# pakozm/lua-mapreduce

Hardware: AMD Instinct MI355X
Metric: words/sec (higher is better)
Workload: dtype u8-text/i64-counts; 1 GPU; model=europarl-wordcount, global_batch=49158635, seq_len=49158635, parallelism=dp1, splits_per_gpu=197, partitions=1, partitioner=hash-mulhi, ingestion=resident-hbm

## Files before the change

### mapreduce_amd/ops/hip/ops_ext.hip

```cpp

#include <ATen/hip/HIPContext.h>
#include <torch/extension.h>

#include <limits>
#include <map>
#include <mutex>
#include <utility>

#include "extract_sorted.hip"
#include "gradsum.hip"
#include "group.hip"
#include "join.hip"
#include "lex_order.hip"
#include "mr_kernels.hip"
#include "postings_phrase.hip"
#include "postings_query.hip"
#include "radix_sort.hip"
#include "seg_scan.hip"
#include "token_ordinals.hip"

namespace {

constexpr int kBlock = 256;
constexpr long kMaxBlocks = 2048;

long grid_for(long n, long per_thread = 1) {
  long want = (n + (long)kBlock * per_thread - 1) / ((long)kBlock * per_thread);
  if (want < 1) want = 1;
  return want < kMaxBlocks ? want : kMaxBlocks;
}

hipStream_t cur_stream() { return at::hip::getCurrentHIPStream(); }

constexpr int kTokWavesPerCu = 16;

struct TokOccupancy {
  int blocks_per_cu = 0;
  int cus = 0;
};

TokOccupancy tok_occupancy(const void* kfn, int blockn) {
  static std::mutex mu;
  static std::map<std::pair<const void*, int>, TokOccupancy> cache;
  int dev = 0;
  C10_HIP_CHECK(hipGetDevice(&dev));
  std::lock_guard<std::mutex> lock(mu);
  auto it = cache.find({kfn, dev});
  if (it != cache.end()) return it->second;
  TokOccupancy o;
  C10_HIP_CHECK(hipOccupancyMaxActiveBlocksPerMultiprocessor(
      &o.blocks_per_cu, kfn, blockn, 0));
  C10_HIP_CHECK(hipDeviceGetAttribute(
      &o.cus, hipDeviceAttributeMultiprocessorCount, dev));
  TORCH_CHECK(o.blocks_per_cu > 0 && o.cus > 0,
              "tokenizer occupancy query returned ", o.blocks_per_cu,
              " blocks/CU on ", o.cus, " CUs");
  cache[{kfn, dev}] = o;
  return o;
}

template <typename K>
long tok_grid(K kfn, int blockn, long n, long tile_bytes) {
  long tiles = (n + tile_bytes - 1) / tile_bytes;
  if (tiles < 1) tiles = 1;
  TokOccupancy o = tok_occupancy(reinterpret_cast<const void*>(kfn), blockn);
  int per_cu = kTokWavesPerCu / (blockn / WAVE);
  if (per_cu > o.blocks_per_cu) per_cu = o.blocks_per_cu;
  long resident = (long)per_cu * o.cus;
  long blocks = tiles < resident ? tiles : resident;
  return blocks < kMaxBlocks ? blocks : kMaxBlocks;
}

int rs_items() {
  static int v = -1;
  if (v < 0) {
    const char* e = getenv("MR_RS_ITEMS");
    const char* v1 = getenv("MR_RADIX_V1");
    v = (e && atoi(e) == 4 && !(v1 && v1[0] == '1')) ? 4 : 8;
  }
  return v;
}

long rs_tile() { return (long)RS_BLOCK * rs_items(); }

bool radix_v1_forced() {
  const char* v = getenv("MR_RADIX_V1");
  return v && v[0] == '1';
}

void launch_radix_hist(const u64* kin, long n, int shift, long ntiles,
                       i64* hist) {
  auto kfn = rs_items() == 4 ? radix_hist_kernel<4> : radix_hist_kernel<8>;
  hipLaunchKernelGGL(kfn, dim3(ntiles), dim3(RS_BLOCK), 0, cur_stream(),
                     kin, n, shift, ntiles, hist);
}

void launch_radix_scatter(const u64* kin, const u64* vin, long n, int shift,
                          long ntiles, const i64* base, u64* kout,
                          u64* vout) {
  static int use_v1 = -1;
  if (use_v1 < 0) use_v1 = radix_v1_forced() ? 1 : 0;
  if (use_v1)
    hipLaunchKernelGGL(radix_scatter_kernel, dim3(ntiles), dim3(RS_BLOCK), 0,
                       cur_stream(), kin, vin, n, shift, ntiles, base, kout,
                       vout);
  else {
    auto kfn = rs_items() == 4 ? radix_scatter_v2_kernel<4>
                               : radix_scatter_v2_kernel<8>;
    hipLaunchKernelGGL(kfn, dim3(ntiles), dim3(RS_BLOCK),
                       0, cur_stream(), kin, vin, n, shift, ntiles, base,
                       kout, vout);
  }
}

void launch_radix_scatter32(const u64* kin, const u32* vin, long n,
                            int shift, long ntiles, const i64* base,
                            u64* kout, u32* vout) {
  auto kfn = rs_items() == 4 ? radix_scatter_v2_kernel<4, u32>
                             : radix_scatter_v2_kernel<8, u32>;
  hipLaunchKernelGGL(kfn, dim3(ntiles), dim3(RS_BLOCK), 0, cur_stream(),
                     kin, vin, n, shift, ntiles, base, kout, vout);
}

template <bool SKIP>
void launch_bucketize_hist(const u64* kin, long n, int shift, long ntiles,
                           u32* hist) {
  auto kfn = rs_items() == 4 ? radix_hist_kernel<4, SKIP, u32>
                             : radix_hist_kernel<8, SKIP, u32>;
  hipLaunchKernelGGL(kfn, dim3(ntiles), dim3(RS_BLOCK), 0, cur_stream(),
                     kin, n, shift, ntiles, hist);
}

template <typename VT, bool SKIP>
void launch_bucketize_scatter(const u64* kin, const VT* vin, long n,
                              int shift, long ntiles, const u32* base,
                              u64* kout, VT* vout) {
  auto kfn = rs_items() == 4 ? radix_scatter_v2_kernel<4, VT, SKIP, u32>
                             : radix_scatter_v2_kernel<8, VT, SKIP, u32>;
  hipLaunchKernelGGL(kfn, dim3(ntiles), dim3(RS_BLOCK), 0, cur_stream(),
                     kin, vin, n, shift, ntiles, base, kout, vout);
}

u64* u64p(torch::Tensor& t) { return reinterpret_cast<u64*>(t.data_ptr<i64>()); }
const u64* u64cp(const torch::Tensor& t) {
  return reinterpret_cast<const u64*>(t.data_ptr<i64>());
}

void check_dev_i64(const torch::Tensor& t, const char* name) {
  TORCH_CHECK(t.is_cuda(), name, " must be on GPU");
  TORCH_CHECK(t.scalar_type() == torch::kInt64, name, " must be int64");
  TORCH_CHECK(t.is_contiguous(), name, " must be contiguous");
}

}

std::vector<torch::Tensor> tokenize(torch::Tensor text, long cap) {
  TORCH_CHECK(text.is_cuda() && text.scalar_type() == torch::kUInt8 &&
              text.is_contiguous(), "text must be contiguous u8 on GPU");
  long n = text.numel();
  auto opts = torch::TensorOptions().device(text.device()).dtype(torch::kInt64);
  auto out_hash = torch::empty({cap}, opts);
  auto out_pos = torch::empty({cap}, opts);
  auto counter = torch::zeros({1}, opts);
  long blocks = grid_for(n, TOK_BYTES);
  hipLaunchKernelGGL(tokenize_kernel, dim3(blocks), dim3(kBlock), 0,
                     cur_stream(), text.data_ptr<u8>(), n, u64p(out_hash),
                     u64p(out_pos),
                     reinterpret_cast<unsigned long long*>(counter.data_ptr<i64>()),
                     cap);
  return {out_hash, out_pos, counter};
}

void tokenize_count(torch::Tensor text, long pos_base, torch::Tensor tkeys,
                    torch::Tensor tvals, torch::Tensor texm,
                    torch::Tensor nwords) {
  TORCH_CHECK(text.is_cuda() && text.scalar_type() == torch::kUInt8 &&
              text.is_contiguous(), "text must be contiguous u8 on GPU");
  long n = text.numel();
  long cap = tkeys.numel();
  TORCH_CHECK((cap & (cap - 1)) == 0, "table capacity must be a power of 2");
  if (!n) return;
  hipLaunchKernelGGL(tokenize_count_kernel, dim3(grid_for(n, TOK_BYTES)),
                     dim3(kBlock), 0, cur_stream(), text.data_ptr<u8>(), n,
                     (u64)pos_base, u64p(tkeys), tvals.data_ptr<i64>(),
                     texm.numel() ? u64p(texm) : nullptr, (u64)(cap - 1),
                     reinterpret_cast<unsigned long long*>(nwords.data_ptr<i64>()));
}

std::vector<torch::Tensor> tokenize_spill_v2(torch::Tensor text,
                                             long pos_base, long cap) {
  TORCH_CHECK(text.is_cuda() && text.scalar_type() == torch::kUInt8 &&
              text.is_contiguous(), "text must be contiguous u8 on GPU");
  long n = text.numel();
  auto opts = torch::TensorOptions().device(text.device()).dtype(torch::kInt64);
  auto out_hash = torch::empty({cap}, opts);
  auto out_pos = torch::empty({cap}, opts);
  auto counter = torch::zeros({1}, opts);
  auto nwords = torch::zeros({1}, opts);
  if (n) {
    auto dummy = torch::empty({16}, opts);
    hipLaunchKernelGGL((tokenize_v6_kernel<16, false, 4096, 0, true>),
                       dim3(grid_for(n, TOK_BYTES)), dim3(kBlock), 0,
                       cur_stream(), text.data_ptr<u8>(), n, (u64)pos_base,
                       u64p(dummy), dummy.data_ptr<i64>(), nullptr,
                       (u64)15, u64p(out_hash), u64p(out_pos),
                       reinterpret_cast<unsigned long long*>(counter.data_ptr<i64>()),
                       cap,
                       reinterpret_cast<unsigned long long*>(nwords.data_ptr<i64>()),
                       nullptr, (const i64*)nullptr, 0, 0L);
  }
  return {out_hash, out_pos, counter, nwords};
}

std::vector<torch::Tensor> tokenize_spill_composite(
    torch::Tensor text, long pos_base, long cap, torch::Tensor split_off,
    long doc_base) {
  TORCH_CHECK(text.is_cuda() && text.scalar_type() == torch::kUInt8 &&
              text.is_contiguous(), "text must be contiguous u8 on GPU");
  check_dev_i64(split_off, "split_off");
  long n = text.numel();
  auto opts = torch::TensorOptions().device(text.device()).dtype(torch::kInt64);
  auto out_hash = torch::empty({cap}, opts);
  auto out_pos = torch::empty({cap}, opts);
  auto counter = torch::zeros({1}, opts);
  auto nwords = torch::zeros({1}, opts);
  if (n) {
    auto dummy = torch::empty({16}, opts);
    hipLaunchKernelGGL((tokenize_v6_kernel<16, false, 4096, 0, true, true>),
                       dim3(grid_for(n, TOK_BYTES)), dim3(kBlock), 0,
                       cur_stream(), text.data_ptr<u8>(), n, (u64)pos_base,
                       u64p(dummy), dummy.data_ptr<i64>(), nullptr,
                       (u64)15, u64p(out_hash), u64p(out_pos),
                       reinterpret_cast<unsigned long long*>(counter.data_ptr<i64>()),
                       cap,
                       reinterpret_cast<unsigned long long*>(nwords.data_ptr<i64>()),
                       nullptr, split_off.data_ptr<i64>(),
                       (int)split_off.numel(), doc_base);
  }
  return {out_hash, out_pos, counter, nwords};
}

void tokenize_cache_spill_composite(
    torch::Tensor text, long pos_base, torch::Tensor tkeys,
    torch::Tensor tvals, torch::Tensor texm, long spill_cap,
    torch::Tensor nwords, torch::Tensor out_hash, torch::Tensor out_pos,
    torch::Tensor counter, torch::Tensor split_off, long doc_base) {
  TORCH_CHECK(text.is_cuda() && text.scalar_type() == torch::kUInt8 &&
              text.is_contiguous(), "text must be contiguous u8 on GPU");
  check_dev_i64(split_off, "split_off");
  long n = text.numel();
  long cap = tkeys.numel();
  TORCH_CHECK((cap & (cap - 1)) == 0, "table capacity must be a power of 2");
  TORCH_CHECK(out_hash.numel() >= spill_cap && out_pos.numel() >= spill_cap,
              "spill arrays too small");
  if (!n) return;
  auto kfn =
      tokenize_v6_kernel<2048, true, 4096, 0, false, true, 2048, 0, 256>;
  long blocks = tok_grid(kfn, kBlock, n, 4096);
  static torch::Tensor cpos_gc;
  long need = blocks * 2048;
  if (!cpos_gc.defined() || cpos_gc.numel() < need ||
      cpos_gc.device() != text.device())
    cpos_gc = torch::empty({need}, torch::TensorOptions()
                                        .device(text.device())
                                        .dtype(torch::kInt64));
  hipLaunchKernelGGL(
      kfn, dim3(blocks), dim3(kBlock), 0, cur_stream(), text.data_ptr<u8>(), n,
      (u64)pos_base, u64p(tkeys), tvals.data_ptr<i64>(),
      texm.numel() ? u64p(texm) : nullptr, (u64)(cap - 1), u64p(out_hash),
      u64p(out_pos),
      reinterpret_cast<unsigned long long*>(counter.data_ptr<i64>()),
      spill_cap,
      reinterpret_cast<unsigned long long*>(nwords.data_ptr<i64>()),
      u64p(cpos_gc), split_off.data_ptr<i64>(), (int)split_off.numel(),
      doc_base);
}

std::vector<torch::Tensor> tokenize_spill(torch::Tensor text, long pos_base,
                                          long cap) {
  TORCH_CHECK(text.is_cuda() && text.scalar_type() == torch::kUInt8 &&
              text.is_contiguous(), "text must be contiguous u8 on GPU");
  long n = text.numel();
  auto opts = torch::TensorOptions().device(text.device()).dtype(torch::kInt64);
  auto out_hash = torch::empty({cap}, opts);
  auto out_pos = torch::empty({cap}, opts);
  auto counter = torch::zeros({1}, opts);
  if (n)
    hipLaunchKernelGGL(tokenize_spill_kernel, dim3(grid_for(n, TOK_BYTES)),
                       dim3(kBlock), 0, cur_stream(), text.data_ptr<u8>(), n,
                       (u64)pos_base, u64p(out_hash), u64p(out_pos),
                       reinterpret_cast<unsigned long long*>(counter.data_ptr<i64>()),
                       cap);
  return {out_hash, out_pos, counter};
}

void tokenize_cache_spill(
    torch::Tensor text, long pos_base, torch::Tensor tkeys,
    torch::Tensor tvals, torch::Tensor texm, long spill_cap,
    torch::Tensor nwords, torch::Tensor out_hash, torch::Tensor out_pos,
    torch::Tensor counter) {
  TORCH_CHECK(text.is_cuda() && text.scalar_type() == torch::kUInt8 &&
              text.is_contiguous(), "text must be contiguous u8 on GPU");
  long n = text.numel();
  long cap = tkeys.numel();
  TORCH_CHECK((cap & (cap - 1)) == 0, "table capacity must be a power of 2");
  TORCH_CHECK(out_hash.numel() >= spill_cap && out_pos.numel() >= spill_cap,
              "spill arrays too small");
  if (n) {
    const char* v = getenv("MR_TOKENIZE_V5");
    const char* v4 = getenv("MR_TOKENIZE_V4");
    if (!(v && v[0] == '1') && !(v4 && v4[0] == '1')) {
      const char* cs = getenv("MR_TOK_CACHE");
      int cache = cs ? atoi(cs) : 2048;
      const char* gp = getenv("MR_TOK_GPOS");
      bool gpos = !(gp && gp[0] == '0');
      const char* ts = getenv("MR_TOK_TILE");
      int tsz = ts ? atoi(ts) : 4096;
      const char* sc = getenv("MR_SPILL_CHUNK");
      int schunk = sc ? atoi(sc) : 2048;
      const char* tb = getenv("MR_TOK_BLOCK");
      int blockn = (tb && atoi(tb) == 512) ? 512 : 256;
      if (blockn == 512) tsz = 8192;
      auto kfn = tokenize_v6_kernel<2048, false, 4096>;
      if (gpos && blockn == 512)
        kfn = tokenize_v6_kernel<2048, true, 8192, 0, false, false, 2048,
                                 0, 512>;
      else if (gpos && tsz == 8192) kfn = tokenize_v6_kernel<2048, true, 8192>;
      else if (gpos && cache == 4096) kfn = tokenize_v6_kernel<4096, true, 4096>;
      else if (gpos && cache == 1024) kfn = tokenize_v6_kernel<1024, true, 4096>;
      else if (gpos && schunk == 128)
        kfn = tokenize_v6_kernel<2048, true, 4096, 0, false, false, 128>;
      else if (gpos && schunk == 1024)
        kfn = tokenize_v6_kernel<2048, true, 4096, 0, false, false, 1024>;
      else if (gpos && schunk == 2048)
        kfn = tokenize_v6_kernel<2048, true, 4096, 0, false, false, 2048>;
      else if (gpos && schunk == 4096)
        kfn = tokenize_v6_kernel<2048, true, 4096, 0, false, false, 4096>;
      else if (gpos) kfn = tokenize_v6_kernel<2048, true, 4096>;
      else if (cache == 512) kfn = tokenize_v6_kernel<512, false, 4096>;
      else if (cache == 1024) kfn = tokenize_v6_kernel<1024, false, 4096>;
      else if (schunk == 128)
        kfn = tokenize_v6_kernel<2048, false, 4096, 0, false, false, 128>;
      long blocks = tok_grid(kfn, blockn, n, tsz);
      static torch::Tensor cpos_g;
      u64* cpg = nullptr;
      if (gpos) {
        long need = blocks * (cache > 2048 ? cache : 2048);
        if (!cpos_g.defined() || cpos_g.numel() < need ||
            cpos_g.device() != text.device())
          cpos_g = torch::empty({need},
                                torch::TensorOptions().device(text.device())
                                    .dtype(torch::kInt64));
        cpg = u64p(cpos_g);
      }
      hipLaunchKernelGGL(kfn,
                         dim3(blocks), dim3(blockn), 0,
                         cur_stream(), text.data_ptr<u8>(), n, (u64)pos_base,
                         u64p(tkeys), tvals.data_ptr<i64>(),
                         texm.numel() ? u64p(texm) : nullptr, (u64)(cap - 1),
                         u64p(out_hash), u64p(out_pos),
                         reinterpret_cast<unsigned long long*>(counter.data_ptr<i64>()),
                         spill_cap,
                         reinterpret_cast<unsigned long long*>(nwords.data_ptr<i64>()),
                         cpg, (const i64*)nullptr, 0, 0L);
    } else if (!(v && v[0] == '1'))
      hipLaunchKernelGGL(tokenize_cache_spill_kernel,
                         dim3(grid_for(n, TOK_BYTES)), dim3(kBlock), 0,
                         cur_stream(), text.data_ptr<u8>(), n, (u64)pos_base,
                         u64p(tkeys), tvals.data_ptr<i64>(),
                         texm.numel() ? u64p(texm) : nullptr, (u64)(cap - 1),
                         u64p(out_hash), u64p(out_pos),
                         reinterpret_cast<unsigned long long*>(counter.data_ptr<i64>()),
                         spill_cap,
                         reinterpret_cast<unsigned long long*>(nwords.data_ptr<i64>()));
    else
      hipLaunchKernelGGL(tokenize_v5_kernel,
                         dim3(grid_for(n, TOK_BYTES)), dim3(kBlock), 0,
                         cur_stream(), text.data_ptr<u8>(), n, (u64)pos_base,
                         u64p(tkeys), tvals.data_ptr<i64>(),
                         texm.numel() ? u64p(texm) : nullptr, (u64)(cap - 1),
                         u64p(out_hash), u64p(out_pos),
                         reinterpret_cast<unsigned long long*>(counter.data_ptr<i64>()),
                         spill_cap,
                         reinterpret_cast<unsigned long long*>(nwords.data_ptr<i64>()));
  }
}

void tokenize_cache_spill_bucketed(
    torch::Tensor text, long pos_base, torch::Tensor tkeys,
    torch::Tensor tvals, torch::Tensor texm, long spill_bcap,
    torch::Tensor nwords, torch::Tensor out_hash, torch::Tensor out_pos,
    torch::Tensor counters) {
  TORCH_CHECK(text.is_cuda() && text.scalar_type() == torch::kUInt8 &&
              text.is_contiguous(), "text must be contiguous u8 on GPU");
  long n = text.numel();
  long cap = tkeys.numel();
  TORCH_CHECK((cap & (cap - 1)) == 0, "table capacity must be a power of 2");
  TORCH_CHECK(counters.numel() >= 256, "counters must hold 256 buckets");
  TORCH_CHECK(out_hash.numel() >= 256 * spill_bcap &&
              out_pos.numel() >= 256 * spill_bcap, "spill arrays too small");
  if (!n) return;
  const char* gp = getenv("MR_TOK_GPOS");
  bool gpos = !(gp && gp[0] == '0');
  auto kfn = tokenize_v6_kernel<2048, false, 4096, 0, false, false, 512, 256>;
  if (gpos)
    kfn = tokenize_v6_kernel<2048, true, 4096, 0, false, false, 512, 256>;
  long blocks = tok_grid(kfn, kBlock, n, 4096);
  static torch::Tensor cpos_gb;
  u64* cpg = nullptr;
  if (gpos) {
    long need = blocks * 2048;
    if (!cpos_gb.defined() || cpos_gb.numel() < need ||
        cpos_gb.device() != text.device())
      cpos_gb = torch::empty({need},
                             torch::TensorOptions().device(text.device())
                                 .dtype(torch::kInt64));
    cpg = u64p(cpos_gb);
  }
  hipLaunchKernelGGL(kfn, dim3(blocks), dim3(kBlock), 0, cur_stream(),
                     text.data_ptr<u8>(), n, (u64)pos_base, u64p(tkeys),
                     tvals.data_ptr<i64>(),
                     texm.numel() ? u64p(texm) : nullptr, (u64)(cap - 1),
                     u64p(out_hash), u64p(out_pos),
                     reinterpret_cast<unsigned long long*>(counters.data_ptr<i64>()),
                     spill_bcap,
                     reinterpret_cast<unsigned long long*>(nwords.data_ptr<i64>()),
                     cpg, (const i64*)nullptr, 0, 0L);
}

double tok6_ablate(torch::Tensor text, long mode, long iters) {
  long n = text.numel();
  auto opts = torch::TensorOptions().device(text.device()).dtype(torch::kInt64);
  long tcap = 1 << 19;
  auto tkeys = torch::full({tcap}, -1, opts);
  auto tvals = torch::zeros({tcap}, opts);
  auto texm = torch::zeros({tcap}, opts);
  long cap = n / 2 + 16;
  auto oh = torch::empty({cap}, opts);
  auto op = torch::empty({cap}, opts);
  auto ctr = torch::zeros({1}, opts);
  auto nw = torch::zeros({1}, opts);
// ... 1203 lines not shown
```

### mapreduce_amd/ops/hip/radix_sort.hip

```cpp

#include "common.h"

#define RS_BLOCK 256
#define RS_WAVES (RS_BLOCK / WAVE)
#define RS_ITEMS 8
#define RS_TILE (RS_BLOCK * RS_ITEMS)
#define RS_BINS 256

template <bool SKIP>
DEV bool rs_live(u64 k) { return !SKIP || k != HT_EMPTY; }

template <int ITEMS, bool SKIP = false, typename HT = i64>
__global__ __launch_bounds__(RS_BLOCK) void radix_hist_kernel(
    const u64* __restrict__ keys, long n, int shift, long ntiles,
    HT* __restrict__ hist) {
  __shared__ u32 lh[RS_BINS];
  for (int b = threadIdx.x; b < RS_BINS; b += blockDim.x) lh[b] = 0;
  __syncthreads();
  long tile = blockIdx.x;
  long base = tile * (RS_BLOCK * ITEMS);
  for (int r = 0; r < ITEMS; ++r) {
    long i = base + r * RS_BLOCK + threadIdx.x;
    if (i < n) {
      u64 k = keys[i];
      if (rs_live<SKIP>(k)) atomicAdd(&lh[(u32)((k >> shift) & 0xFF)], 1u);
    }
  }
  __syncthreads();
  for (int b = threadIdx.x; b < RS_BINS; b += blockDim.x)
    hist[(long)b * ntiles + tile] = (HT)lh[b];
}

template <int ITEMS, typename VT = u64, bool SKIP = false, typename BT = i64>
__global__ __launch_bounds__(RS_BLOCK) void radix_scatter_v2_kernel(
    const u64* __restrict__ keys, const VT* __restrict__ vals, long n,
    int shift, long ntiles, const BT* __restrict__ base_dx,
    u64* __restrict__ okeys, VT* __restrict__ ovals) {
  __shared__ u32 wavecnt[RS_WAVES][RS_BINS];
  __shared__ u32 cnt_base[RS_BINS];
  __shared__ u32 digit_start[RS_BINS + 1];
  __shared__ u64 stage_k[(RS_BLOCK * ITEMS)];
  __shared__ VT stage_v[(RS_BLOCK * ITEMS)];
  for (int b = threadIdx.x; b < RS_BINS; b += blockDim.x) cnt_base[b] = 0;
  long tile = blockIdx.x;
  long tbase = tile * (RS_BLOCK * ITEMS);
  long tile_n = n - tbase < (RS_BLOCK * ITEMS) ? n - tbase : (RS_BLOCK * ITEMS);
  int wave = threadIdx.x / WAVE;
  int lane = threadIdx.x % WAVE;
  u64 lt_mask = ((u64)1 << lane) - 1;
  bool has_vals = ovals != nullptr;

  __syncthreads();
  for (int r = 0; r < ITEMS; ++r) {
    long i = tbase + (long)r * RS_BLOCK + threadIdx.x;
    if (i < n) {
      u64 k = keys[i];
      if (rs_live<SKIP>(k))
        atomicAdd(&cnt_base[(u32)((k >> shift) & 0xFF)], 1u);
    }
  }
  __syncthreads();
  if (threadIdx.x == 0) {
    u32 run = 0;
    for (int d = 0; d < RS_BINS; ++d) {
      digit_start[d] = run;
      run += cnt_base[d];
    }
    digit_start[RS_BINS] = run;
  }
  __syncthreads();
  for (int b = threadIdx.x; b < RS_BINS; b += blockDim.x) cnt_base[b] = 0;
  __syncthreads();

  for (int r = 0; r < ITEMS; ++r) {
    for (int b = threadIdx.x; b < RS_BINS; b += blockDim.x)
      for (int w = 0; w < RS_WAVES; ++w) wavecnt[w][b] = 0;
    __syncthreads();
    long i = tbase + (long)r * RS_BLOCK + threadIdx.x;
    bool valid = i < n;
    u64 k = valid ? keys[i] : 0;
    valid = valid && rs_live<SKIP>(k);
    u32 d = valid ? (u32)((k >> shift) & 0xFF) : 0;
    u64 m = __ballot(valid);
    #pragma unroll
    for (int b = 0; b < 8; ++b) {
      u64 bb = __ballot(valid && ((d >> b) & 1));
      m &= ((d >> b) & 1) ? bb : ~bb;
    }
    u32 lane_rank = 0;
    if (valid) {
      lane_rank = (u32)__popcll(m & lt_mask);
      int leader = __ffsll((unsigned long long)m) - 1;
      if (lane == leader) wavecnt[wave][d] = (u32)__popcll(m);
    }
    __syncthreads();
    if (threadIdx.x < RS_BINS) {
      u32 run = cnt_base[threadIdx.x];
      #pragma unroll
      for (int w = 0; w < RS_WAVES; ++w) {
        u32 c = wavecnt[w][threadIdx.x];
        wavecnt[w][threadIdx.x] = run;
        run += c;
      }
      cnt_base[threadIdx.x] = run;
    }
    __syncthreads();
    if (valid) {
      u32 s = digit_start[d] + wavecnt[wave][d] + lane_rank;
      stage_k[s] = k;
      if (has_vals) stage_v[s] = vals[i];
    }
    __syncthreads();
  }

  long nstage = SKIP ? (long)digit_start[RS_BINS] : tile_n;
  for (long s = threadIdx.x; s < nstage; s += blockDim.x) {
    u64 k = stage_k[s];
    u32 d = (u32)((k >> shift) & 0xFF);
    u32 local = (u32)s - digit_start[d];
    long pos = (long)base_dx[(long)d * ntiles + tile] + local;
    okeys[pos] = k;
    if (has_vals) ovals[pos] = stage_v[s];
  }
}

__global__ __launch_bounds__(RS_BLOCK) void radix_scatter_kernel(
    const u64* __restrict__ keys, const u64* __restrict__ vals, long n,
    int shift, long ntiles, const i64* __restrict__ base_dx,
    u64* __restrict__ okeys, u64* __restrict__ ovals) {
  __shared__ u32 wavecnt[RS_WAVES][RS_BINS];
  __shared__ u32 cnt_base[RS_BINS];
  for (int b = threadIdx.x; b < RS_BINS; b += blockDim.x) cnt_base[b] = 0;
  long tile = blockIdx.x;
  long tbase = tile * RS_TILE;
  int wave = threadIdx.x / WAVE;
  int lane = threadIdx.x % WAVE;
  u64 lt_mask = ((u64)1 << lane) - 1;

  for (int r = 0; r < RS_ITEMS; ++r) {
    for (int b = threadIdx.x; b < RS_BINS; b += blockDim.x)
      for (int w = 0; w < RS_WAVES; ++w) wavecnt[w][b] = 0;
    __syncthreads();

    long i = tbase + (long)r * RS_BLOCK + threadIdx.x;
    bool valid = i < n;
    u64 k = valid ? keys[i] : 0;
    u32 d = valid ? (u32)((k >> shift) & 0xFF) : 0;

    u64 m = __ballot(valid);
    #pragma unroll
    for (int b = 0; b < 8; ++b) {
      u64 bb = __ballot(valid && ((d >> b) & 1));
      m &= ((d >> b) & 1) ? bb : ~bb;
    }
    u32 lane_rank = 0;
    if (valid) {
      lane_rank = (u32)__popcll(m & lt_mask);
      int leader = __ffsll((unsigned long long)m) - 1;
      if (lane == leader) wavecnt[wave][d] = (u32)__popcll(m);
    }
    __syncthreads();

    if (threadIdx.x < RS_BINS) {
      u32 run = cnt_base[threadIdx.x];
      #pragma unroll
      for (int w = 0; w < RS_WAVES; ++w) {
        u32 c = wavecnt[w][threadIdx.x];
        wavecnt[w][threadIdx.x] = run;
        run += c;
      }
      cnt_base[threadIdx.x] = run;
    }
    __syncthreads();

    if (valid) {
      u32 tile_rank = wavecnt[wave][d] + lane_rank;
      long pos = base_dx[(long)d * ntiles + tile] + tile_rank;
      okeys[pos] = k;
      if (ovals) ovals[pos] = vals[i];
    }
    __syncthreads();
  }
}

#define RS_SCAN_UNROLL 4

DEV u32 wave_incl_scan_u32(u32 v, int lane) {
  #pragma unroll
  for (int off = 1; off < WAVE; off <<= 1) {
    u32 o = __shfl_up(v, off, WAVE);
    if (lane >= off) v += o;
  }
  return v;
}

__global__ __launch_bounds__(RS_BLOCK) void rs_row_totals_kernel(
    const u32* __restrict__ hist, long ntiles, i64* __restrict__ totals) {
  __shared__ i64 wsum[RS_WAVES];
  const u32* row = hist + (long)blockIdx.x * ntiles;
  i64 acc = 0;
  for (long t0 = threadIdx.x; t0 < ntiles; t0 += RS_SCAN_UNROLL * RS_BLOCK) {
    u32 v[RS_SCAN_UNROLL];
    #pragma unroll
    for (int j = 0; j < RS_SCAN_UNROLL; ++j) {
      long t = t0 + (long)j * RS_BLOCK;
      v[j] = t < ntiles ? row[t] : 0;
    }
    #pragma unroll
    for (int j = 0; j < RS_SCAN_UNROLL; ++j) acc += v[j];
  }
  acc = wave_sum_i64(acc);
  if (threadIdx.x % WAVE == 0) wsum[threadIdx.x / WAVE] = acc;
  __syncthreads();
  if (threadIdx.x == 0) {
    i64 s = 0;
    for (int w = 0; w < RS_WAVES; ++w) s += wsum[w];
    totals[blockIdx.x] = s;
  }
}

__global__ __launch_bounds__(RS_BLOCK) void rs_row_scan_kernel(
    u32* __restrict__ hist, long ntiles, const i64* __restrict__ totals,
    i64* __restrict__ bucket_off) {
  __shared__ i64 wsum[RS_WAVES];
  __shared__ u32 wpre[RS_SCAN_UNROLL * RS_WAVES];
  __shared__ i64 row_base;
  int d = blockIdx.x;
  int wave = threadIdx.x / WAVE;
  int lane = threadIdx.x % WAVE;
  i64 tv = totals[threadIdx.x];
  i64 part = wave_sum_i64(threadIdx.x < d ? tv : 0);
  if (lane == 0) wsum[wave] = part;
  __syncthreads();
  if (threadIdx.x == 0) {
    i64 s = 0;
    for (int w = 0; w < RS_WAVES; ++w) s += wsum[w];
    row_base = s;
    bucket_off[d] = s;
    if (d == RS_BINS - 1) bucket_off[RS_BINS] = s + totals[d];
  }
  __syncthreads();
  u32 carry = (u32)row_base;
  u32* row = hist + (long)d * ntiles;
  for (long t0 = 0; t0 < ntiles; t0 += RS_SCAN_UNROLL * RS_BLOCK) {
    u32 v[RS_SCAN_UNROLL], inc[RS_SCAN_UNROLL];
    #pragma unroll
    for (int j = 0; j < RS_SCAN_UNROLL; ++j) {
      long t = t0 + (long)j * RS_BLOCK + threadIdx.x;
      v[j] = t < ntiles ? row[t] : 0;
    }
    #pragma unroll
    for (int j = 0; j < RS_SCAN_UNROLL; ++j) {
      inc[j] = wave_incl_scan_u32(v[j], lane);
      if (lane == WAVE - 1) wpre[j * RS_WAVES + wave] = inc[j];
    }
    __syncthreads();
    u32 run = carry;
    #pragma unroll
    for (int j = 0; j < RS_SCAN_UNROLL; ++j) {
      #pragma unroll
      for (int w = 0; w < RS_WAVES; ++w) {
        if (w == wave) {
          long t = t0 + (long)j * RS_BLOCK + threadIdx.x;
          if (t < ntiles) row[t] = run + inc[j] - v[j];
        }
        run += wpre[j * RS_WAVES + w];
      }
    }
    carry = run;
    __syncthreads();
  }
}

__global__ __launch_bounds__(256) void gather_i64_u32_kernel(
    const i64* __restrict__ vals, const u32* __restrict__ idx, long n,
    i64* __restrict__ out) {
  long i = (long)blockIdx.x * blockDim.x + threadIdx.x;
  long stride = (long)gridDim.x * blockDim.x;
  for (; i < n; i += stride) out[i] = vals[idx[i]];
}
```

Measured before the change: 42.60 billion words/s.

## Add single-pass register-resident radix scatter kernel and vectorized histogram loads

Adds a v3 radix scatter kernel that loads all tile keys into registers once and ranks them per wave with ballot-based match masks. Each thread owns one digit for the block-wide scan, and the kernel stages the keys in shared memory sorted by digit so the global writes land contiguously. This replaces the v2 kernel's repeated per-round block barriers and its second read of the keys. The bucketize histogram also gains a 16-byte vector load path for full, aligned tiles. The old behaviour stays available through MR_RADIX_V2=1. The cost is higher register and LDS pressure, which could lower occupancy.

Result: faster. 49.33 billion words/s (median of 6 runs) (+15.8%).

```diff
diff --git a/mapreduce_amd/ops/hip/ops_ext.hip b/mapreduce_amd/ops/hip/ops_ext.hip
--- a/mapreduce_amd/ops/hip/ops_ext.hip
+++ b/mapreduce_amd/ops/hip/ops_ext.hip
@@ -88,6 +88,22 @@
   return v && v[0] == '1';
 }
 
+bool radix_v2_forced() {
+  static int f = -1;
+  if (f < 0) {
+    const char* v = getenv("MR_RADIX_V2");
+    f = (v && v[0] == '1') ? 1 : 0;
+  }
+  return f == 1;
+}
+
+#define RS_STAGED_SCATTER(VT, SKIP, BT, LATE)                              \
+  (radix_v2_forced()                                                       \
+       ? (rs_items() == 4 ? radix_scatter_v2_kernel<4, VT, SKIP, BT>       \
+                          : radix_scatter_v2_kernel<8, VT, SKIP, BT>)      \
+       : (rs_items() == 4 ? radix_scatter_v3_kernel<4, VT, SKIP, BT, LATE> \
+                          : radix_scatter_v3_kernel<8, VT, SKIP, BT, LATE>))
+
 void launch_radix_hist(const u64* kin, long n, int shift, long ntiles,
                        i64* hist) {
   auto kfn = rs_items() == 4 ? radix_hist_kernel<4> : radix_hist_kernel<8>;
@@ -105,8 +121,7 @@
                        cur_stream(), kin, vin, n, shift, ntiles, base, kout,
                        vout);
   else {
-    auto kfn = rs_items() == 4 ? radix_scatter_v2_kernel<4>
-                               : radix_scatter_v2_kernel<8>;
+    auto kfn = RS_STAGED_SCATTER(u64, false, i64, true);
     hipLaunchKernelGGL(kfn, dim3(ntiles), dim3(RS_BLOCK),
                        0, cur_stream(), kin, vin, n, shift, ntiles, base,
                        kout, vout);
@@ -116,8 +131,7 @@
 void launch_radix_scatter32(const u64* kin, const u32* vin, long n,
                             int shift, long ntiles, const i64* base,
                             u64* kout, u32* vout) {
-  auto kfn = rs_items() == 4 ? radix_scatter_v2_kernel<4, u32>
-                             : radix_scatter_v2_kernel<8, u32>;
+  auto kfn = RS_STAGED_SCATTER(u32, false, i64, true);
   hipLaunchKernelGGL(kfn, dim3(ntiles), dim3(RS_BLOCK), 0, cur_stream(),
                      kin, vin, n, shift, ntiles, base, kout, vout);
 }
@@ -125,8 +139,11 @@
 template <bool SKIP>
 void launch_bucketize_hist(const u64* kin, long n, int shift, long ntiles,
                            u32* hist) {
-  auto kfn = rs_items() == 4 ? radix_hist_kernel<4, SKIP, u32>
-                             : radix_hist_kernel<8, SKIP, u32>;
+  auto kfn = rs_items() == 4 ? radix_hist_kernel<4, SKIP, u32, true>
+                             : radix_hist_kernel<8, SKIP, u32, true>;
+  if (radix_v2_forced())
+    kfn = rs_items() == 4 ? radix_hist_kernel<4, SKIP, u32>
+                          : radix_hist_kernel<8, SKIP, u32>;
   hipLaunchKernelGGL(kfn, dim3(ntiles), dim3(RS_BLOCK), 0, cur_stream(),
                      kin, n, shift, ntiles, hist);
 }
@@ -135,8 +152,7 @@
 void launch_bucketize_scatter(const u64* kin, const VT* vin, long n,
                               int shift, long ntiles, const u32* base,
                               u64* kout, VT* vout) {
-  auto kfn = rs_items() == 4 ? radix_scatter_v2_kernel<4, VT, SKIP, u32>
-                             : radix_scatter_v2_kernel<8, VT, SKIP, u32>;
+  auto kfn = RS_STAGED_SCATTER(VT, SKIP, u32, false);
   hipLaunchKernelGGL(kfn, dim3(ntiles), dim3(RS_BLOCK), 0, cur_stream(),
                      kin, vin, n, shift, ntiles, base, kout, vout);
 }
diff --git a/mapreduce_amd/ops/hip/radix_sort.hip b/mapreduce_amd/ops/hip/radix_sort.hip
--- a/mapreduce_amd/ops/hip/radix_sort.hip
+++ b/mapreduce_amd/ops/hip/radix_sort.hip
@@ -10,7 +10,7 @@
 template <bool SKIP>
 DEV bool rs_live(u64 k) { return !SKIP || k != HT_EMPTY; }
 
-template <int ITEMS, bool SKIP = false, typename HT = i64>
+template <int ITEMS, bool SKIP = false, typename HT = i64, bool WIDE = false>
 __global__ __launch_bounds__(RS_BLOCK) void radix_hist_kernel(
     const u64* __restrict__ keys, long n, int shift, long ntiles,
     HT* __restrict__ hist) {
@@ -19,11 +19,26 @@
   __syncthreads();
   long tile = blockIdx.x;
   long base = tile * (RS_BLOCK * ITEMS);
-  for (int r = 0; r < ITEMS; ++r) {
-    long i = base + r * RS_BLOCK + threadIdx.x;
-    if (i < n) {
-      u64 k = keys[i];
-      if (rs_live<SKIP>(k)) atomicAdd(&lh[(u32)((k >> shift) & 0xFF)], 1u);
+  if (WIDE && base + RS_BLOCK * ITEMS <= n &&
+      ((unsigned long long)keys & 15) == 0) {
+    const ulonglong2* p = reinterpret_cast<const ulonglong2*>(keys + base);
+    ulonglong2 q[ITEMS / 2];
+    #pragma unroll
+    for (int j = 0; j < ITEMS / 2; ++j) q[j] = p[j * RS_BLOCK + threadIdx.x];
+    #pragma unroll
+    for (int j = 0; j < ITEMS / 2; ++j) {
+      if (rs_live<SKIP>(q[j].x))
+        atomicAdd(&lh[(u32)((q[j].x >> shift) & 0xFF)], 1u);
+      if (rs_live<SKIP>(q[j].y))
+        atomicAdd(&lh[(u32)((q[j].y >> shift) & 0xFF)], 1u);
+    }
+  } else {
+    for (int r = 0; r < ITEMS; ++r) {
+      long i = base + r * RS_BLOCK + threadIdx.x;
+      if (i < n) {
+        u64 k = keys[i];
+        if (rs_live<SKIP>(k)) atomicAdd(&lh[(u32)((k >> shift) & 0xFF)], 1u);
+      }
     }
   }
   __syncthreads();
@@ -124,6 +139,145 @@
   }
 }
 
+DEV u32 wave_incl_scan_u32(u32 v, int lane) {
+  #pragma unroll
+  for (int off = 1; off < WAVE; off <<= 1) {
+    u32 o = __shfl_up(v, off, WAVE);
+    if (lane >= off) v += o;
+  }
+  return v;
+}
+
+template <int ITEMS, typename VT = u64, bool SKIP = false, typename BT = i64,
+          bool LATE = false>
+__global__ __launch_bounds__(RS_BLOCK) void radix_scatter_v3_kernel(
+    const u64* __restrict__ keys, const VT* __restrict__ vals, long n,
+    int shift, long ntiles, const BT* __restrict__ base_dx,
+    u64* __restrict__ okeys, VT* __restrict__ ovals) {
+  static_assert(RS_BLOCK == RS_BINS, "thread b owns digit b");
+  __shared__ u32 wcnt[RS_WAVES][RS_BINS];
+  __shared__ BT gbase[RS_BINS];
+  __shared__ u64 stage_k[(RS_BLOCK * ITEMS)];
+  __shared__ VT stage_v[(RS_BLOCK * ITEMS)];
+  long tile = blockIdx.x;
+  long tbase = tile * (RS_BLOCK * ITEMS);
+  long tile_n = n - tbase < (RS_BLOCK * ITEMS) ? n - tbase : (RS_BLOCK * ITEMS);
+  int wave = threadIdx.x / WAVE;
+  int lane = threadIdx.x % WAVE;
+  u64 lt_mask = ((u64)1 << lane) - 1;
+  bool has_vals = ovals != nullptr;
+
+  BT my_base = base_dx[(long)threadIdx.x * ntiles + tile];
+  long i0 = tbase + (long)(wave * ITEMS) * WAVE + lane;
+  u64 k[ITEMS];
+  VT v[ITEMS];
+  bool valid[ITEMS];
+  #pragma unroll
+  for (int r = 0; r < ITEMS; ++r) {
+    long i = i0 + (long)r * WAVE;
+    k[r] = keys[i < n ? i : n - 1];
+  }
+  if (has_vals && !LATE) {
+    #pragma unroll
+    for (int r = 0; r < ITEMS; ++r) {
+      long i = i0 + (long)r * WAVE;
+      v[r] = vals[i < n ? i : n - 1];
+    }
+  } else {
+    #pragma unroll
+    for (int r = 0; r < ITEMS; ++r) v[r] = 0;
+  }
+  #pragma unroll
+  for (int r = 0; r < ITEMS; ++r)
+    valid[r] = i0 + (long)r * WAVE < n && rs_live<SKIP>(k[r]);
+
+  #pragma unroll
+  for (int b = lane; b < RS_BINS; b += WAVE) wcnt[wave][b] = 0;
+  __builtin_amdgcn_fence(__ATOMIC_ACQ_REL, "wavefront");
+  __builtin_amdgcn_wave_barrier();
+  u32 rank[ITEMS];
+  #pragma unroll
+  for (int r = 0; r < ITEMS; ++r) {
+    u32 d = valid[r] ? (u32)((k[r] >> shift) & 0xFF) : 0;
+    u64 m = __ballot(valid[r]);
+    #pragma unroll
+    for (int b = 0; b < 8; ++b) {
+      u64 bb = __ballot(valid[r] && ((d >> b) & 1));
+      m &= ((d >> b) & 1) ? bb : ~bb;
+    }
+    u32 prev = valid[r] ? wcnt[wave][d] : 0;
+    rank[r] = prev + (u32)__popcll(m & lt_mask);
+    __builtin_amdgcn_fence(__ATOMIC_ACQ_REL, "wavefront");
+    __builtin_amdgcn_wave_barrier();
+    if (valid[r] && lane == __ffsll((unsigned long long)m) - 1)
+      wcnt[wave][d] = prev + (u32)__popcll(m);
+    __builtin_amdgcn_fence(__ATOMIC_ACQ_REL, "wavefront");
+    __builtin_amdgcn_wave_barrier();
+  }
+  __syncthreads();
+
+  u32 wb[RS_WAVES];
+  u32 total = 0;
+  #pragma unroll
+  for (int w = 0; w < RS_WAVES; ++w) {
+    wb[w] = total;
+    total += wcnt[w][threadIdx.x];
+  }
+  u32 incl = wave_incl_scan_u32(total, lane);
+  if (lane == WAVE - 1) stage_k[wave] = incl;
+  __syncthreads();
+  u32 pre = 0, all = 0;
+  #pragma unroll
+  for (int w = 0; w < RS_WAVES; ++w) {
+    u32 ws = (u32)stage_k[w];
+    if (w < wave) pre += ws;
+    all += ws;
+  }
+  u32 dstart = pre + incl - total;
+  #pragma unroll
+  for (int w = 0; w < RS_WAVES; ++w) wcnt[w][threadIdx.x] = dstart + wb[w];
+  gbase[threadIdx.x] = my_base - (BT)dstart;
+  __syncthreads();
+
+  #pragma unroll
+  for (int r = 0; r < ITEMS; ++r) {
+    u32 d = (u32)((k[r] >> shift) & 0xFF);
+    rank[r] += valid[r] ? wcnt[wave][d] : 0;
+  }
+  #pragma unroll
+  for (int r = 0; r < ITEMS; ++r) {
+    if (valid[r]) {
+      stage_k[rank[r]] = k[r];
+      if (has_vals)
+        stage_v[rank[r]] = LATE ? vals[i0 + (long)r * WAVE] : v[r];
+    }
+  }
+  __syncthreads();
+
+  u32 nstage = SKIP ? all : (u32)tile_n;
+  long pos[ITEMS];
+  #pragma unroll
+  for (int j = 0; j < ITEMS; ++j) {
+    u32 s = j * RS_BLOCK + threadIdx.x;
+    k[j] = s < nstage ? stage_k[s] : 0;
+    if (has_vals) v[j] = s < nstage ? stage_v[s] : (VT)0;
+  }
+  #pragma unroll
+  for (int j = 0; j < ITEMS; ++j) {
+    u32 s = j * RS_BLOCK + threadIdx.x;
+    u32 d = (u32)((k[j] >> shift) & 0xFF);
+    pos[j] = (long)(BT)(gbase[d] + (BT)s);
+  }
+  #pragma unroll
+  for (int j = 0; j < ITEMS; ++j) {
+    u32 s = j * RS_BLOCK + threadIdx.x;
+    if (s < nstage) {
+      okeys[pos[j]] = k[j];
+      if (has_vals) ovals[pos[j]] = v[j];
+    }
+  }
+}
+
 __global__ __launch_bounds__(RS_BLOCK) void radix_scatter_kernel(
     const u64* __restrict__ keys, const u64* __restrict__ vals, long n,
     int shift, long ntiles, const i64* __restrict__ base_dx,
@@ -185,15 +339,6 @@
 
 #define RS_SCAN_UNROLL 4
 
-DEV u32 wave_incl_scan_u32(u32 v, int lane) {
-  #pragma unroll
-  for (int off = 1; off < WAVE; off <<= 1) {
-    u32 o = __shfl_up(v, off, WAVE);
-    if (lane >= off) v += o;
-  }
-  return v;
-}
-
 __global__ __launch_bounds__(RS_BLOCK) void rs_row_totals_kernel(
     const u32* __restrict__ hist, long ntiles, i64* __restrict__ totals) {
   __shared__ i64 wsum[RS_WAVES];
```
